# peteroh23/ModulationDetectionCNN

Measured on AMD Instinct MI355X. Metric: I/Q frames/sec (2x128, VT-CNN2, batch=2^20), higher is better.
Workload: dtype bf16; 1 GPU; vtcnn2-c11-bf16-n2^20; topology=vtcnn2, classes=11, frames_per_gpu=1048576, global_batch=1048576, parallelism=batch-shard x1 (no collective), outputs=softmax probabilities f32 + argmax int32, frames_per_forward_call=1048576, full=False

## Files before the change

### modulationdetectioncnn_amd/csrc/mdc_api.hip

```cpp
#include "mdc_internal.h"

#include <cstdlib>
#include <cstring>
#include <exception>
#include <mutex>
#include <new>

namespace mdc {

static thread_local char g_err[512] = "";

void set_error(const char* fmt, ...) {
    va_list ap;
    va_start(ap, fmt);
    vsnprintf(g_err, sizeof(g_err), fmt, ap);
    va_end(ap);
}

int upload(mdc_model* m, int idx, const void* host, size_t bytes) {
    if (m->d_pack[idx]) {
        (void)hipFree(m->d_pack[idx]);
        m->d_pack[idx] = nullptr;
    }
    MDC_HIP(hipMalloc(&m->d_pack[idx], bytes));
// ... 71 lines not shown
            return MDC_EINVAL;
    }
}

extern "C" {

int mdc_abi_version(void) { return MDC_ABI_VERSION; }

const char* mdc_last_error(void) { return g_err; }

int mdc_create(const mdc_topology* topo, int device, mdc_model** out) {
    return guarded("mdc_create", [&]() -> int {
        if (!topo || !out) { set_error("mdc_create: null argument"); return MDC_EINVAL; }
        *out = nullptr;
        if ((topo->reserved[0] & ~MDC_OPT_ALL) != 0) { set_error("mdc_create: unknown option bits 0x%x in reserved[0]", topo->reserved[0]); return MDC_EINVAL; }
        for (int i = 1; i < 4; ++i) if (topo->reserved[i] != 0) { set_error("mdc_create: reserved[1..3] must be 0"); return MDC_EINVAL; }
        if ((topo->reserved[0] & MDC_OPT_FP8_BF16_FEATURES) && topo->kind != MDC_KIND_VTCNN2) {
            set_error("mdc_create: MDC_OPT_FP8_BF16_FEATURES applies to MDC_KIND_VTCNN2 only");
            return MDC_EINVAL;
        }
        int ndev = 0;
        if (hipGetDeviceCount(&ndev) != hipSuccess || ndev == 0) { set_error("no HIP device available"); return MDC_ENODEV; }
        if (device < 0 || device >= ndev) { set_error("device %d out of range (have %d)", device, ndev); return MDC_ENODEV; }
        hipDeviceProp_t prop;
        MDC_HIP(hipGetDeviceProperties(&prop, device));
        if (std::strncmp(prop.gcnArchName, "gfx950", 6) != 0) {
            set_error("device %d is %s; libmdc.so carries gfx950 (MI355X) code only", device, prop.gcnArchName);
            return MDC_ENODEV;
        }
        mdc_model* m = new (std::nothrow) mdc_model();
        if (!m) { set_error("out of host memory"); return MDC_ENOMEM; }
        m->topo = *topo;
        m->device = device;
#ifdef MDC_ALTERNATES
        {
            auto flag = [](const char* name, int when) { const char* e = getenv(name); return e && atoi(e) == when; };
            if (flag("MDC_CONV_SCHED", 0)) m->alt |= kAltConvHipcc;
            if (flag("MDC_DENSE1_PHASED", 0)) m->alt |= kAltDense1Simple;
            if (flag("MDC_DEP_F32_MFMA", 1)) m->alt |= kAltDepF32Mfma;
            if (flag("MDC_D1_FUSED_HEAD", 0)) m->alt |= kAltSeparateHead;
            if (const char* e = getenv("MDC_DEP_RING")) m->alt_ring = atoi(e);
        }
#endif
        int rc = MDC_ENOMEM;
        try { rc = layer_layout(m); } catch (...) { delete m; throw; }
        if (rc != MDC_OK) { delete m; return rc; }
        *out = m;
        return MDC_OK;
    });
}

int mdc_num_layers(const mdc_model* m) {
    if (!m) { set_error("null model"); return MDC_EINVAL; }
    return m->nlayers;
}

int mdc_layer_sizes(const mdc_model* m, int layer, size_t* kernel_elems, size_t* bias_elems) {
    if (!m || layer < 0 || layer >= m->nlayers) { set_error("mdc_layer_sizes: bad layer %d", layer); return MDC_EINVAL; }
    if (kernel_elems) *kernel_elems = m->nk[layer];
    if (bias_elems) *bias_elems = m->nb[layer];
    return MDC_OK;
}

int mdc_set_weights(mdc_model* m, int layer, const float* kernel_host, size_t kernel_elems,
                    const float* bias_host, size_t bias_elems) {
    return guarded("mdc_set_weights", [&]() -> int {
        if (!m || !kernel_host || !bias_host) { set_error("mdc_set_weights: null argument"); return MDC_EINVAL; }
        if (m->finalized) { set_error("mdc_set_weights: model is finalized (immutable)"); return MDC_ESTATE; }
        if (layer < 0 || layer >= m->nlayers) { set_error("mdc_set_weights: layer %d out of range 0..%d", layer, m->nlayers - 1); return MDC_EINVAL; }
        if (kernel_elems != m->nk[layer] || bias_elems != m->nb[layer]) {
            set_error("mdc_set_weights: layer %d expects kernel %zu / bias %zu elements, got %zu / %zu",
                      layer, m->nk[layer], m->nb[layer], kernel_elems, bias_elems);
            return MDC_EINVAL;
        }
// ... 322 lines not shown
```

### modulationdetectioncnn_amd/csrc/mdc_internal.h

```cpp
#pragma once
#include <hip/hip_runtime.h>
#include <cstdarg>
#include <cstdint>
#include <cstdio>
#include <exception>
#include <mutex>
#include <new>
#include <string>
#include <type_traits>
#include <vector>

#include "mdc.h"

namespace mdc {

void set_error(const char* fmt, ...);

template <class Fn>
inline int guarded(const char* what, Fn&& fn) noexcept {
    try {
        return fn();
    } catch (const std::bad_alloc&) {
        set_error("%s: out of host memory", what);
        return MDC_ENOMEM;
// ... 55 lines not shown
    return max(max(__float_as_uint(v.x) & 0x7FFFFFFFu, __float_as_uint(v.y) & 0x7FFFFFFFu),
               max(__float_as_uint(v.z) & 0x7FFFFFFFu, __float_as_uint(v.w) & 0x7FFFFFFFu));
}

enum { kAltConvHipcc = 1,
       kAltDense1Simple = 2,
       kAltDepF32Mfma = 4,
       kAltSeparateHead = 8 };

struct ProfSlot {
    const char* name;
    std::vector<hipEvent_t> ev;
    double total_ms = 0;
    int64_t launches = 0;
};

}

struct mdc_model {
    mdc_topology topo{};
    int device = 0;
    int dtype = MDC_F32;
    bool finalized = false;
    int nlayers = 0;
    size_t nk[4]{}, nb[4]{};
    std::vector<float> hk[4], hb[4];
    bool have[4]{};

    void* d_pack[8]{};
    size_t pack_bytes[8]{};

    int alt = 0;
    int alt_ring = -1;
    float fp8_input_absmax = 0.02f;
    float fp8_feature_absmax = 0.f;
    int fp8_feat_scale_log2 = 0;
    bool fp8_e4m3_features = false;
    float fp8_feat_divisor = 1.f;
    int feat_scale_log2 = 0;

    bool profiling = false;
    std::vector<mdc::ProfSlot> slots;
    std::mutex prof_mu;

    void* host_ctx = nullptr;
    std::mutex host_mu;
};

namespace mdc {

struct ProfScope {
    mdc_model* m;
    int slot;
    hipStream_t s;
    hipEvent_t start = nullptr;
    ProfScope(const mdc_model* mm, int slot_, hipStream_t s_);
    ~ProfScope();
    ProfScope(const ProfScope&) = delete;
    ProfScope& operator=(const ProfScope&) = delete;
};

int upload(mdc_model* m, int idx, const void* host, size_t bytes);

struct DeviceScope {
    int prev = -1, want;
    bool ok = true;
// ... 67 lines not shown
```

### modulationdetectioncnn_amd/csrc/vtcnn2_bf16_common.h

```cpp
#pragma once
#include "mdc_internal.h"

#include <cstring>

namespace mdc {

using f32x4 = __attribute__((ext_vector_type(4))) float;
using f32x2 = __attribute__((ext_vector_type(2))) float;
using bf16x8 = __attribute__((ext_vector_type(8))) __bf16;
using bf16x2 = __attribute__((ext_vector_type(2))) __bf16;
using s16x4 = __attribute__((ext_vector_type(4))) short;
using s16x2 = __attribute__((ext_vector_type(2))) short;
using u32x4 = __attribute__((ext_vector_type(4))) unsigned;
using u32x2 = __attribute__((ext_vector_type(2))) unsigned;

namespace {

constexpr int kPairs = 67;
constexpr int kImgWords = 2 * kPairs * 64;
constexpr int kPartFloats = 4 * 5 * 64 * 4;
constexpr size_t kConvBf16Lds = (size_t)2 * kImgWords * 4 + (size_t)2 * kPartFloats * 4 + 512;
constexpr int kWFrags = 2 * 3 * 2 * 5;

__device__ __forceinline__ unsigned pack2(float a, float b) {
// ... 37 lines not shown
#pragma unroll
    for (int e = 0; e < 2; ++e) {
        const float a = xs[2 * e], b = xs[2 * e + 1];
        const unsigned hi = pack2(a, b);
        const float ah = __uint_as_float(hi << 16), bh = __uint_as_float(hi & 0xFFFF0000u);
        const unsigned lo = pack2(a - ah, b - bh);
        unsigned* d = im + (h * kPairs + 2 * m + 1 + e) * 64 + i;
        d[0] = hi;
        d[16] = lo;
        d[32] = hi;
    }
}
template <bool U8 = false>
__device__ __forceinline__ void stage_quarter(int k, const float* __restrict__ x, long n, long frame0,
                                              unsigned* __restrict__ im, int tid, long hop2 = 256, float scale = 0.f) {
    stage_write(k, stage_decode<U8>(stage_load<U8>(k, x, n, frame0, tid, hop2), tid, scale), n, frame0, im, tid);
}

__device__ __forceinline__ void glds16(const void* gsrc, void* lds_wave_base) {
    __builtin_amdgcn_global_load_lds((const __attribute__((address_space(1))) void*)gsrc,
                                     (__attribute__((address_space(3))) void*)lds_wave_base, 16, 0, 0);
}

__device__ __forceinline__ void glds16_nt(const void* gsrc, void* lds_wave_base) {
    __builtin_amdgcn_global_load_lds((const __attribute__((address_space(1))) void*)gsrc,
                                     (__attribute__((address_space(3))) void*)lds_wave_base, 16, 0, 2);
}

__device__ __forceinline__ void glds16_async(const void* gsrc, void* lds_wave_base) {
    const unsigned l = (unsigned)(size_t)(__attribute__((address_space(3))) unsigned char*)lds_wave_base;
    asm volatile("global_load_lds_dwordx4 %0, off" ::"v"(gsrc), "{m0}"(l) : "memory");
}

inline unsigned short f2bf(float f) {
    unsigned u;
    std::memcpy(&u, &f, 4);
    if ((u & 0x7F800000u) == 0x7F800000u) return (unsigned short)(u >> 16);
    u += 0x7FFFu + ((u >> 16) & 1u);
    return (unsigned short)(u >> 16);
}
inline float bf2f(unsigned short h) {
    unsigned u = (unsigned)h << 16;
    float f;
    std::memcpy(&f, &u, 4);
    return f;
}

}

int vtcnn2_bf16_conv_sched(const mdc_model* m, const float* x, int64_t n, void* feat, hipStream_t s, long hop2 = 0, float scale = 0.f);
int vtcnn2_bf16_pack_sched(mdc_model* m);

}
```

### modulationdetectioncnn_amd/csrc/vtcnn2_bf16_dense1.hip

```cpp
#include "vtcnn2_bf16_common.h"
#include "dense_chain_common.h"

#include <cstdlib>

namespace mdc {

namespace {

constexpr int kBM = 256, kBN = 256, kBK = 64;
constexpr int kTileBytes = kBM * kBK * 2;
constexpr size_t kDenseBf16Lds = (size_t)4 * kTileBytes;
constexpr size_t kDenseHeadLds = (size_t)128 * kChainXld * 4;
static_assert(kDenseHeadLds >= kDenseBf16Lds, "the fused-head form allocates the larger of the two");
constexpr int kNT = kFeat / kBK;

__device__ __forceinline__ bf16x8 cvt_e4m3x8(u32x2 r) {
    const bf16x2 p0 = __builtin_amdgcn_cvt_scalef32_pk_bf16_fp8(r[0], 1.0f, false);
    const bf16x2 p1 = __builtin_amdgcn_cvt_scalef32_pk_bf16_fp8(r[0], 1.0f, true);
    const bf16x2 p2 = __builtin_amdgcn_cvt_scalef32_pk_bf16_fp8(r[1], 1.0f, false);
    const bf16x2 p3 = __builtin_amdgcn_cvt_scalef32_pk_bf16_fp8(r[1], 1.0f, true);
    return bf16x8{p0[0], p0[1], p1[0], p1[1], p2[0], p2[1], p3[0], p3[1]};
}


#if defined(MDC_ALTERNATES) || defined(MDC_ABLATIONS)
template <int ABL>
__global__ __launch_bounds__(512) void vt_dense1_bf16_kernel(const unsigned short* __restrict__ feat, long n,
                                                             const unsigned short* __restrict__ w1t,
                                                             const float* __restrict__ c1,
                                                             float* __restrict__ hid) {
    extern __shared__ __attribute__((aligned(16))) unsigned char smem[];
    const int tid = threadIdx.x, lane = tid & 63;
    const int wv = __builtin_amdgcn_readfirstlane(tid >> 6);
    const int wr = wv >> 2, wc = wv & 3;
    const int fr = lane & 15, fg = lane >> 4;
    const long row0 = (long)blockIdx.x * kBM;

    const int srow = lane >> 3, spos = lane & 7;
    const unsigned short* asrc[4];
    const unsigned short* bsrc[4];
#pragma unroll
    for (int p = 0; p < 4; ++p) {
        const int r = (wv * 4 + p) * 8 + srow;
        long gr = (ABL == 1 ? 0 : row0) + r;
        if (gr >= n) gr = n - 1;
// ... 46 lines not shown
                for (int j = 0; j < 4; ++j)
                    acc[i][j] = __builtin_amdgcn_mfma_f32_16x16x32_bf16(af[i], bfr[j], acc[i][j], 0, 0, 0);
        }
    };

    stage(0, 0);
    __syncthreads();
    int cur = 0;
    for (int t = 0; t < kNT - 1; ++t) {
        stage(t + 1, cur ^ 1);
        compute(cur);
        __syncthreads();
        cur ^= 1;
    }
    compute(cur);

#pragma unroll
    for (int j = 0; j < 4; ++j) {
        const int col = wc * 64 + j * 16 + fr;
        const float bias = c1[col];
#pragma unroll
        for (int i = 0; i < 8; ++i)
#pragma unroll
            for (int r = 0; r < 4; ++r) {
                const long row = row0 + wr * 128 + i * 16 + fg * 4 + r;
                if (row < n) hid[row * kHid + col] = fmaxf(acc[i][j][r] + bias, 0.f);
            }
    }
}


#endif

template <bool HEAD>
__device__ __forceinline__ void d1_epilogue(f32x4 (&acc)[8][4], unsigned char* smem, long row0, long n, int lane, int wv,
                                            const float* __restrict__ c1, float* __restrict__ hid, const float* __restrict__ w2pack,
                                            int n_out, float* __restrict__ probs, int* __restrict__ labels) {
    const int wr = wv >> 2, wc = wv & 3, fr = lane & 15, fg = lane >> 4;
    if constexpr (!HEAD) {
#pragma unroll
        for (int j = 0; j < 4; ++j) {
            const int col = wc * 64 + j * 16 + fr;
            const float bias = c1[col];
#pragma unroll
            for (int i = 0; i < 8; ++i)
#pragma unroll
                for (int r = 0; r < 4; ++r) {
                    const long row = row0 + wr * 128 + i * 16 + fg * 4 + r;
                    if (row < n) hid[row * kHid + col] = fmaxf(acc[i][j][r] + bias, 0.f);
                }
        }
    } else {
        float* xs = reinterpret_cast<float*>(smem);
        float w2[64];
#pragma unroll
        for (int i = 0; i < 64; ++i) w2[i] = w2pack[i * 64 + lane];
        const float b2 = w2pack[64 * 64 + 16 * 64 + fr];
        float bias1[4];
#pragma unroll
        for (int j = 0; j < 4; ++j) bias1[j] = c1[wc * 64 + j * 16 + fr];
#pragma unroll
        for (int half = 0; half < 2; ++half) {
            __syncthreads();
            if (wr == half) {
#pragma unroll
                for (int j = 0; j < 4; ++j)
#pragma unroll
                    for (int i = 0; i < 8; ++i)
#pragma unroll
                        for (int r = 0; r < 4; ++r)
                            xs[(i * 16 + fg * 4 + r) * kChainXld + wc * 64 + j * 16 + fr] = fmaxf(acc[i][j][r] + bias1[j], 0.f);
            }
            __syncthreads();
            const f32x4 a2 = chain_k256(xs + (wv * 16 + fr) * kChainXld + fg, w2, f32x4{0.f, 0.f, 0.f, 0.f});
            f32x4 z;
#pragma unroll
            for (int r = 0; r < 4; ++r) z[r] = a2[r] + b2;
            chain_softmax_store(z, fr, fg, row0 + half * 128 + wv * 16, n, n_out, probs, labels, nullptr);
        }
    }
}

constexpr int kUnitBytes = 128 * 128;

template <int ABL, bool HEAD = false, bool F8 = false>
__global__ __launch_bounds__(512) void vt_dense1_bf16_phased_kernel(const unsigned short* __restrict__ feat, long n,
                                                                    const unsigned short* __restrict__ w1t,
                                                                    const float* __restrict__ c1, float* __restrict__ hid,
                                                                    const float* __restrict__ w2pack = nullptr, int n_out = 0,
                                                                    float* __restrict__ probs = nullptr, int* __restrict__ labels = nullptr) {
    extern __shared__ __attribute__((aligned(16))) unsigned char smem[];
    const int tid = threadIdx.x, lane = tid & 63;
    const int wv = __builtin_amdgcn_readfirstlane(tid >> 6);
    const int wr = wv >> 2, wc = wv & 3;
    const int fr = lane & 15, fg = lane >> 4;
    const long row0 = (long)blockIdx.x * kBM;

    const int srow = lane >> 3, spos = lane & 7;
    const unsigned short* src[4][2];
#pragma unroll
    for (int j = 0; j < 2; ++j) {
        const int u = (wv * 2 + j) * 8 + srow;
        const int sw = (spos ^ (u & 7)) * 8;
        const int arow_lo = 128 * (u >> 6) + (u & 63);
        const int brow_lo = 64 * (u >> 5) + (u & 31);
        long g0 = (ABL == 1 ? 0 : row0) + arow_lo, g3 = (ABL == 1 ? 0 : row0) + arow_lo + 64;
        if (g0 >= n) g0 = n - 1;
        if (g3 >= n) g3 = n - 1;
        src[0][j] = feat + g0 * (long)kFeat + sw;
        src[3][j] = feat + g3 * (long)kFeat + sw;
        src[1][j] = w1t + brow_lo * kBK + sw;
        src[2][j] = w1t + (brow_lo + 32) * kBK + sw;
    }
    const unsigned char* src8[2] = {nullptr, nullptr};
    if constexpr (F8) {
        const int u = wv * 16 + (lane >> 2);
        const int sw = ((lane & 3) ^ ((u >> 2) & 3)) * 16;
        const int arow_lo = 128 * (u >> 6) + (u & 63);
        long g0 = row0 + arow_lo, g3 = row0 + arow_lo + 64;
        if (g0 >= n) g0 = n - 1;
        if (g3 >= n) g3 = n - 1;
        const unsigned char* f8 = reinterpret_cast<const unsigned char*>(feat);
        src8[0] = f8 + g0 * (long)kFeat + sw;
        src8[1] = f8 + g3 * (long)kFeat + sw;
    }
    auto stage_unit = [&](int t, int unit, int b) {
        if (ABL == 2 && (unit == 1 || unit == 2) && (t & 1)) return;
        unsigned char* dst = smem + ((size_t)b * 4 + unit) * kUnitBytes + (wv * 2) * 1024;
        if constexpr (F8) {
            if (unit == 0 || unit == 3) {
                glds16(src8[unit == 3] + (long)t * kBK, smem + ((size_t)b * 4 + unit) * kUnitBytes + wv * 1024);
                return;
            }
        }
        if (unit == 0 || unit == 3) {
            glds16_nt(src[unit][0] + (long)t * kBK, dst);
            glds16_nt(src[unit][1] + (long)t * kBK, dst + 1024);
        } else {
            glds16(src[unit][0] + (long)t * (kBN * kBK), dst);
            glds16(src[unit][1] + (long)t * (kBN * kBK), dst + 1024);
        }
    };

    auto frag = [&](const unsigned char* unit_base, int u, int ks) {
        return *reinterpret_cast<const bf16x8*>(unit_base + u * 128 + (((ks * 4 + fg) ^ (u & 7)) * 16));
    };

    f32x4 acc[8][4];
#pragma unroll
    for (int i = 0; i < 8; ++i)
#pragma unroll
        for (int j = 0; j < 4; ++j) acc[i][j] = f32x4{0.f, 0.f, 0.f, 0.f};
    bf16x8 a0[4][2], a1[4][2], b0[2][2], b1[2][2];
    u32x2 ra[4][2];

    unsigned ra_lane[2] = {0u, 0u};
    if constexpr (F8) {
        ra_lane[0] = (unsigned)((64 * wr + fr) * 64 + ((((fg >> 1) ^ ((fr >> 2) & 3)) * 16) + (fg & 1) * 8));
        ra_lane[1] = ra_lane[0] ^ 32u;
    }
    auto read_a = [&](bf16x8 (&a)[4][2], int unit, int b) {
        if (ABL == 3 && b == 1) return;
        const unsigned char* base = smem + ((size_t)b * 4 + unit) * kUnitBytes;
        if constexpr (F8) {
            const unsigned bl = (unsigned)(size_t)(__attribute__((address_space(3))) unsigned char*)const_cast<unsigned char*>(base);
            const unsigned ad0 = bl + ra_lane[0], ad1 = bl + ra_lane[1];
#pragma unroll
            for (int i = 0; i < 4; ++i) {
                asm volatile("ds_read_b64 %0, %1 offset:%2" : "=v"(ra[i][0]) : "v"(ad0), "i"(i * 1024) : "memory");
                asm volatile("ds_read_b64 %0, %1 offset:%2" : "=v"(ra[i][1]) : "v"(ad1), "i"(i * 1024) : "memory");
            }
        } else {
#pragma unroll
            for (int i = 0; i < 4; ++i)
#pragma unroll
                for (int ks = 0; ks < 2; ++ks) a[i][ks] = frag(base, 64 * wr + 16 * i + fr, ks);
        }
    };
    auto cvt_a = [&](bf16x8 (&a)[4][2]) {
        if constexpr (F8) {
#pragma unroll
            for (int i = 0; i < 4; ++i)
#pragma unroll
                for (int ks = 0; ks < 2; ++ks) a[i][ks] = cvt_e4m3x8(ra[i][ks]);
        }
// ... 18 lines not shown
                for (int j = 0; j < 2; ++j)
                    acc[i0 + i][j0 + j] = __builtin_amdgcn_mfma_f32_16x16x32_bf16(a[i][ks], bq[j][ks], acc[i0 + i][j0 + j], 0, 0, 0);
#ifndef D1_NOPRIO
        __builtin_amdgcn_s_setprio(0);
#endif
    };
    auto quadrant_cv = [&](bf16x8 (&a)[4][2], const bf16x8 (&bq)[2][2], int i0, int j0, bf16x8 (&dst)[4][2], auto own) {
        constexpr bool OWN = decltype(own)::value;
        __builtin_amdgcn_s_setprio(1);
        if constexpr (OWN) a[0][0] = cvt_e4m3x8(ra[0][0]);
#pragma unroll
        for (int f = 0; f < 8; ++f) {
            const int ks = f >> 2, i = f & 3;
            if constexpr (OWN) { if (f + 1 < 8) a[(f + 1) & 3][(f + 1) >> 2] = cvt_e4m3x8(ra[(f + 1) & 3][(f + 1) >> 2]); }
            else dst[i][ks] = cvt_e4m3x8(ra[i][ks]);
#pragma unroll
            for (int j = 0; j < 2; ++j)
                acc[i0 + i][j0 + j] = __builtin_amdgcn_mfma_f32_16x16x32_bf16(a[i][ks], bq[j][ks], acc[i0 + i][j0 + j], 0, 0, 0);
        }
        if constexpr (OWN) __builtin_amdgcn_sched_group_barrier(0x002, 4, 0);
#pragma unroll
        for (int f = 0; f < 16; ++f) {
            __builtin_amdgcn_sched_group_barrier(0x008, 1, 0);
            __builtin_amdgcn_sched_group_barrier(0x002, 2, 0);
        }
        __builtin_amdgcn_s_setprio(0);
    };
#define D1_WAIT_BARRIER(N) do { asm volatile("s_waitcnt vmcnt(" #N ")" ::: "memory"); __builtin_amdgcn_s_barrier(); } while (0)
#define D1_LGKM() asm volatile("s_waitcnt lgkmcnt(0)" ::: "memory")
#define D1_LGKM_RA() asm volatile("s_waitcnt lgkmcnt(0)" : "+v"(ra[0][0]), "+v"(ra[0][1]), "+v"(ra[1][0]), "+v"(ra[1][1]), \
                                  "+v"(ra[2][0]), "+v"(ra[2][1]), "+v"(ra[3][0]), "+v"(ra[3][1]) :: "memory")

#pragma unroll
    for (int u = 0; u < 4; ++u) stage_unit(0, u, 0);
    D1_WAIT_BARRIER(0);
    read_a(a0, 0, 0);
    if constexpr (F8) { D1_LGKM_RA(); cvt_a(a0); }
#ifndef D1_NOSTAGGER
    if (wr == 1) __builtin_amdgcn_s_barrier();
#endif

    for (int t = 0; t < kNT; ++t) {
        const int b = t & 1;
        const bool more = t + 1 < kNT;
        if (more) stage_unit(t + 1, 0, b ^ 1);
        __builtin_amdgcn_sched_barrier(0);
        read_b(b0, 1, b);
        if constexpr (F8) { if (more) D1_WAIT_BARRIER(2); else D1_WAIT_BARRIER(1); }
        else { if (more) D1_WAIT_BARRIER(4); else D1_WAIT_BARRIER(2); }
        D1_LGKM();
        quadrant(a0, b0, 0, 0);
        __builtin_amdgcn_s_barrier();
        if (more) stage_unit(t + 1, 1, b ^ 1);
        __builtin_amdgcn_sched_barrier(0);
        read_b(b1, 2, b);
        if constexpr (F8) { if (more) D1_WAIT_BARRIER(3); else D1_WAIT_BARRIER(0); }
        else { if (more) D1_WAIT_BARRIER(4); else D1_WAIT_BARRIER(0); }
        D1_LGKM();
        quadrant(a0, b1, 0, 2);
        __builtin_amdgcn_s_barrier();
        if (more) stage_unit(t + 1, 2, b ^ 1);
        __builtin_amdgcn_sched_barrier(0);
        read_a(a1, 3, b);
        if (more) D1_WAIT_BARRIER(4); else __builtin_amdgcn_s_barrier();
        if constexpr (F8) { D1_LGKM_RA(); quadrant_cv(a1, b1, 4, 2, a1, std::true_type{}); }
        else { D1_LGKM(); quadrant(a1, b1, 4, 2); }
        __builtin_amdgcn_s_barrier();
        if (more) stage_unit(t + 1, 3, b ^ 1);
        __builtin_amdgcn_sched_barrier(0);
        if (more) read_a(a0, 0, b ^ 1);
        if constexpr (F8) { if (more) D1_WAIT_BARRIER(3); else __builtin_amdgcn_s_barrier(); }
        else { if (more) D1_WAIT_BARRIER(4); else __builtin_amdgcn_s_barrier(); }
        if constexpr (F8) {
            if (more) { D1_LGKM_RA(); quadrant_cv(a1, b0, 4, 0, a0, std::false_type{}); }
            else { D1_LGKM(); quadrant(a1, b0, 4, 0); }
        } else {
            quadrant(a1, b0, 4, 0);
            D1_LGKM();
        }
        __builtin_amdgcn_s_barrier();
    }
#ifndef D1_NOSTAGGER
    if (wr == 0) __builtin_amdgcn_s_barrier();
#endif
#undef D1_WAIT_BARRIER
#undef D1_LGKM
#undef D1_LGKM_RA

    d1_epilogue<HEAD>(acc, smem, row0, n, lane, wv, c1, hid, w2pack, n_out, probs, labels);
}


template <bool F8>
__global__ __launch_bounds__(64) void vt_dense1_bf16_small_kernel(const unsigned short* __restrict__ feat, long n,
                                                                  const unsigned short* __restrict__ w1t,
                                                                  const float* __restrict__ c1, float* __restrict__ hid) {
    const int lane = threadIdx.x, fr = lane & 15, fg = lane >> 4;
    const long row0 = (long)blockIdx.x * 16;
    const int col0 = blockIdx.y * 16;
    long ar = row0 + fr;
    if (ar >= n) ar = n - 1;
    using AFrag = typename std::conditional<F8, u32x2, bf16x8>::type;
    const unsigned char* ap = reinterpret_cast<const unsigned char*>(feat) + (ar * (long)kFeat + fg * 8) * (F8 ? 1 : 2);
    const unsigned short* bp = w1t + (long)(col0 + fr) * kBK + fg * 8;
    f32x4 acc = f32x4{0.f, 0.f, 0.f, 0.f};
    constexpr int kU = 5, kBlocks = kNT / kU;
    static_assert(kNT % kU == 0 && kBlocks % 2 == 1, "blocks: an even count in the loop, the last one drained after it");
    AFrag a0[kU][2], a1[kU][2];
    bf16x8 b0[kU][2], b1[kU][2];
    auto load = [&](AFrag (&af)[kU][2], bf16x8 (&bfr)[kU][2], int blk) {
#pragma unroll
        for (int u = 0; u < kU; ++u)
#pragma unroll
            for (int ks = 0; ks < 2; ++ks) {
                af[u][ks] = *reinterpret_cast<const AFrag*>(ap + ((blk * kU + u) * kBK + ks * 32) * (F8 ? 1 : 2));
                bfr[u][ks] = *reinterpret_cast<const bf16x8*>(bp + (long)(blk * kU + u) * (kBN * kBK) + ks * 32);
            }
    };
    auto mma = [&](const AFrag (&af)[kU][2], const bf16x8 (&bfr)[kU][2]) {
#pragma unroll
        for (int u = 0; u < kU; ++u)
#pragma unroll
            for (int ks = 0; ks < 2; ++ks) {
// ... 94 lines not shown
        asm volatile("s_waitcnt vmcnt(%0)\n\ts_barrier" ::"n"((kAhead - 1) * kGrp) : "memory");
        read(nxt, g + 1);
        mma(cur, kGrp);
        asm volatile("s_waitcnt lgkmcnt(0)" ::: "memory");
    };
    static_assert(kGroups % 2 == 1 && kTail >= 0 && kTail < kGrp, "pairs of steps, a last full group, then the tail tiles");
    for (int g = 0; g < kGroups - 1; g += 2) {
        step(f0, f1, g);
        step(f1, f0, g + 1);
    }
    step(f0, f1, kGroups - 1);
    mma(f1, kTail);
    asm volatile("s_waitcnt vmcnt(0)" ::: "memory");
    if (wv != 0) return;
    const int col = col0 + fr;
    const float bias = c1[col];
#pragma unroll
    for (int r = 0; r < 4; ++r) {
        const long row = row0 + fg * 4 + r;
        if (row < n) hid[row * kHid + col] = fmaxf(acc[r] + bias, 0.f);
    }
}

constexpr long kCoopBatch = 256;

constexpr long kSmallBatch = 2048;

}

int vtcnn2_bf16_dense1(const mdc_model* m, const void* feat, int64_t n, float* hid, hipStream_t s,
                       bool fuse_head, float* probs, int32_t* labels, bool* fused) {
    if (fused) *fused = false;
    const bool f8 = m->dtype == MDC_FP8 && m->fp8_e4m3_features;
    if (n <= kCoopBatch) {
#define MDC_LAUNCH_COOP(F) do { \
        MDC_HIP(hipFuncSetAttribute(reinterpret_cast<const void*>(vt_dense1_bf16_coop_kernel<F>), hipFuncAttributeMaxDynamicSharedMemorySize, (int)kCoopLds)); \
        hipLaunchKernelGGL(vt_dense1_bf16_coop_kernel<F>, dim3((unsigned)((n + 15) / 16), kHid / 16), dim3(256), kCoopLds, s, \
                           static_cast<const unsigned short*>(feat), (long)n, static_cast<const unsigned short*>(m->d_pack[3]), \
                           static_cast<const float*>(m->d_pack[4]), hid); } while (0)
        if (f8) MDC_LAUNCH_COOP(true); else MDC_LAUNCH_COOP(false);
#undef MDC_LAUNCH_COOP
        MDC_HIP(hipGetLastError());
        return MDC_OK;
    }
    if (n <= kSmallBatch) {
#define MDC_LAUNCH_SMALL(F) hipLaunchKernelGGL(vt_dense1_bf16_small_kernel<F>, dim3((unsigned)((n + 15) / 16), kHid / 16), dim3(64), 0, s, \
                           static_cast<const unsigned short*>(feat), (long)n, static_cast<const unsigned short*>(m->d_pack[3]), \
                           static_cast<const float*>(m->d_pack[4]), hid)
        if (f8) MDC_LAUNCH_SMALL(true); else MDC_LAUNCH_SMALL(false);
#undef MDC_LAUNCH_SMALL
        MDC_HIP(hipGetLastError());
        return MDC_OK;
    }
    const unsigned short* f = static_cast<const unsigned short*>(feat);
    const unsigned short* w1t = static_cast<const unsigned short*>(m->d_pack[3]);
    const float* c1 = static_cast<const float*>(m->d_pack[4]);
    const dim3 grid((unsigned)((n + kBM - 1) / kBM));
#if defined(MDC_ALTERNATES) || defined(MDC_ABLATIONS)
#define MDC_LAUNCH_D1(A) do { \
    MDC_HIP(hipFuncSetAttribute(reinterpret_cast<const void*>(vt_dense1_bf16_kernel<A>), hipFuncAttributeMaxDynamicSharedMemorySize, (int)kDenseBf16Lds)); \
    hipLaunchKernelGGL(vt_dense1_bf16_kernel<A>, grid, dim3(512), kDenseBf16Lds, s, f, (long)n, w1t, c1, hid); } while (0)
#endif
#ifdef MDC_ABLATIONS
    static const int abl = getenv("MDC_ABLATE_D1") ? atoi(getenv("MDC_ABLATE_D1")) : 0;
#define MDC_LAUNCH_PROBE(A) do { \
        MDC_HIP(hipFuncSetAttribute(reinterpret_cast<const void*>(vt_dense1_bf16_phased_kernel<A>), hipFuncAttributeMaxDynamicSharedMemorySize, (int)kDenseBf16Lds)); \
        hipLaunchKernelGGL(vt_dense1_bf16_phased_kernel<A>, grid, dim3(512), kDenseBf16Lds, s, f, (long)n, w1t, c1, hid); \
        MDC_HIP(hipGetLastError()); \
        return MDC_OK; } while (0)
    if (!f8 && abl == 10) MDC_LAUNCH_PROBE(0);
    if (!f8 && abl == 11) MDC_LAUNCH_PROBE(1);
    if (!f8 && abl == 12) MDC_LAUNCH_PROBE(2);
    if (!f8 && abl == 13) MDC_LAUNCH_PROBE(3);
#undef MDC_LAUNCH_PROBE
    if (abl >= 1 && abl <= 3) {
        switch (abl) { case 1: MDC_LAUNCH_D1(1); break; case 2: MDC_LAUNCH_D1(2); break; default: MDC_LAUNCH_D1(3); }
        MDC_HIP(hipGetLastError());
        return MDC_OK;
    }
#endif
#ifdef MDC_ALTERNATES
    if (!f8 && (m->alt & kAltDense1Simple)) {
        MDC_LAUNCH_D1(0);
        MDC_HIP(hipGetLastError());
        return MDC_OK;
    }
    if (m->alt & kAltSeparateHead) fuse_head = false;
#endif
#undef MDC_LAUNCH_D1
#define MDC_LAUNCH_PHASED(F) do { \
    if (fuse_head && (probs || labels)) { \
        MDC_HIP(hipFuncSetAttribute(reinterpret_cast<const void*>(vt_dense1_bf16_phased_kernel<0, true, F>), hipFuncAttributeMaxDynamicSharedMemorySize, (int)kDenseHeadLds)); \
        hipLaunchKernelGGL((vt_dense1_bf16_phased_kernel<0, true, F>), grid, dim3(512), kDenseHeadLds, s, f, (long)n, w1t, c1, hid, \
                           static_cast<const float*>(m->d_pack[5]), (int)m->topo.classes, probs, labels); \
        if (fused) *fused = true; \
    } else { \
        MDC_HIP(hipFuncSetAttribute(reinterpret_cast<const void*>(vt_dense1_bf16_phased_kernel<0, false, F>), hipFuncAttributeMaxDynamicSharedMemorySize, (int)kDenseBf16Lds)); \
        hipLaunchKernelGGL((vt_dense1_bf16_phased_kernel<0, false, F>), grid, dim3(512), kDenseBf16Lds, s, f, (long)n, w1t, c1, hid); \
    } } while (0)
    if (f8) MDC_LAUNCH_PHASED(true); else MDC_LAUNCH_PHASED(false);
#undef MDC_LAUNCH_PHASED
    MDC_HIP(hipGetLastError());
    return MDC_OK;
}

}
```

Measured before the change: 41.78 million frames/s.

## Make dense1 a persistent CU-sized grid that prefetches the next tile during the epilogue

The dense1 GEMM kernel now launches one workgroup per CU and loops over row tiles instead of launching one workgroup per tile. During each tile's epilogue it asynchronously issues the first k-tile loads for the next tile, using non-temporal loads for the feature rows, so the epilogue stores overlap the next tile's loads. The fused head stages W2, b2 and c1 into LDS once per workgroup and splits the head into four 64-row quarters handled by the first row of waves. This cuts per-tile launch and prologue cost, but a single workgroup per CU loses the latency hiding that multiple resident blocks gave, the reserved LDS grows, and only half the waves do head work.

```diff
diff --git a/modulationdetectioncnn_amd/csrc/mdc_api.hip b/modulationdetectioncnn_amd/csrc/mdc_api.hip
--- a/modulationdetectioncnn_amd/csrc/mdc_api.hip
+++ b/modulationdetectioncnn_amd/csrc/mdc_api.hip
@@ -127,6 +127,7 @@
         if (!m) { set_error("out of host memory"); return MDC_ENOMEM; }
         m->topo = *topo;
         m->device = device;
+        m->cu_count = prop.multiProcessorCount;
 #ifdef MDC_ALTERNATES
         {
             auto flag = [](const char* name, int when) { const char* e = getenv(name); return e && atoi(e) == when; };
@@ -135,6 +136,7 @@
             if (flag("MDC_DEP_F32_MFMA", 1)) m->alt |= kAltDepF32Mfma;
             if (flag("MDC_D1_FUSED_HEAD", 0)) m->alt |= kAltSeparateHead;
             if (const char* e = getenv("MDC_DEP_RING")) m->alt_ring = atoi(e);
+            if (const char* e = getenv("MDC_D1_GRID")) m->alt_d1_grid = atoi(e) > 0 ? atoi(e) : 0;
         }
 #endif
         int rc = MDC_ENOMEM;
diff --git a/modulationdetectioncnn_amd/csrc/mdc_internal.h b/modulationdetectioncnn_amd/csrc/mdc_internal.h
--- a/modulationdetectioncnn_amd/csrc/mdc_internal.h
+++ b/modulationdetectioncnn_amd/csrc/mdc_internal.h
@@ -111,6 +111,8 @@
 
     int alt = 0;
     int alt_ring = -1;
+    int alt_d1_grid = 0;
+    int cu_count = 0;
     float fp8_input_absmax = 0.02f;
     float fp8_feature_absmax = 0.f;
     int fp8_feat_scale_log2 = 0;
diff --git a/modulationdetectioncnn_amd/csrc/vtcnn2_bf16_common.h b/modulationdetectioncnn_amd/csrc/vtcnn2_bf16_common.h
--- a/modulationdetectioncnn_amd/csrc/vtcnn2_bf16_common.h
+++ b/modulationdetectioncnn_amd/csrc/vtcnn2_bf16_common.h
@@ -93,6 +93,11 @@
     asm volatile("global_load_lds_dwordx4 %0, off" ::"v"(gsrc), "{m0}"(l) : "memory");
 }
 
+__device__ __forceinline__ void glds16_async_nt(const void* gsrc, void* lds_wave_base) {
+    const unsigned l = (unsigned)(size_t)(__attribute__((address_space(3))) unsigned char*)lds_wave_base;
+    asm volatile("global_load_lds_dwordx4 %0, off nt" ::"v"(gsrc), "{m0}"(l) : "memory");
+}
+
 inline unsigned short f2bf(float f) {
     unsigned u;
     std::memcpy(&u, &f, 4);
diff --git a/modulationdetectioncnn_amd/csrc/vtcnn2_bf16_dense1.hip b/modulationdetectioncnn_amd/csrc/vtcnn2_bf16_dense1.hip
--- a/modulationdetectioncnn_amd/csrc/vtcnn2_bf16_dense1.hip
+++ b/modulationdetectioncnn_amd/csrc/vtcnn2_bf16_dense1.hip
@@ -10,7 +10,10 @@
 constexpr int kBM = 256, kBN = 256, kBK = 64;
 constexpr int kTileBytes = kBM * kBK * 2;
 constexpr size_t kDenseBf16Lds = (size_t)4 * kTileBytes;
-constexpr size_t kDenseHeadLds = (size_t)128 * kChainXld * 4;
+constexpr size_t kDenseHeadOff = (size_t)2 * kTileBytes;
+constexpr size_t kDenseHeadConstOff = kDenseHeadOff + (size_t)64 * kChainXld * 4;
+constexpr int kHeadW2 = 64 * 64, kHeadB2 = 16;
+constexpr size_t kDenseHeadLds = kDenseHeadConstOff + (size_t)(kHeadW2 + kHeadB2 + kHid) * 4;
 static_assert(kDenseHeadLds >= kDenseBf16Lds, "the fused-head form allocates the larger of the two");
 constexpr int kNT = kFeat / kBK;
 
@@ -123,99 +126,126 @@
 
 #endif
 
-template <bool HEAD>
+__device__ __forceinline__ void d1_head_consts(unsigned char* smem, int tid, const float* __restrict__ c1, const float* __restrict__ w2pack) {
+    float* cs = reinterpret_cast<float*>(smem + kDenseHeadConstOff);
+#pragma unroll
+    for (int i = 0; i < kHeadW2 / 512; ++i) cs[i * 512 + tid] = w2pack[i * 512 + tid];
+    if (tid < kHeadB2) cs[kHeadW2 + tid] = w2pack[64 * 64 + 16 * 64 + tid];
+    if (tid < kHid) cs[kHeadW2 + kHeadB2 + tid] = c1[tid];
+    asm volatile("s_waitcnt lgkmcnt(0)" ::: "memory");
+}
+
+template <bool HEAD, class Prefetch>
 __device__ __forceinline__ void d1_epilogue(f32x4 (&acc)[8][4], unsigned char* smem, long row0, long n, int lane, int wv,
                                             const float* __restrict__ c1, float* __restrict__ hid, const float* __restrict__ w2pack,
-                                            int n_out, float* __restrict__ probs, int* __restrict__ labels) {
+                                            int n_out, float* __restrict__ probs, int* __restrict__ labels, Prefetch&& prefetch) {
     const int wr = wv >> 2, wc = wv & 3, fr = lane & 15, fg = lane >> 4;
+    float bias1[4];
     if constexpr (!HEAD) {
+#pragma unroll
+        for (int j = 0; j < 4; ++j) bias1[j] = c1[wc * 64 + j * 16 + fr];
+        asm volatile("" : "+v"(bias1[0]), "+v"(bias1[1]), "+v"(bias1[2]), "+v"(bias1[3]));
+        prefetch();
 #pragma unroll
         for (int j = 0; j < 4; ++j) {
             const int col = wc * 64 + j * 16 + fr;
-            const float bias = c1[col];
 #pragma unroll
             for (int i = 0; i < 8; ++i)
 #pragma unroll
                 for (int r = 0; r < 4; ++r) {
                     const long row = row0 + wr * 128 + i * 16 + fg * 4 + r;
-                    if (row < n) hid[row * kHid + col] = fmaxf(acc[i][j][r] + bias, 0.f);
+                    if (row < n) hid[row * kHid + col] = fmaxf(acc[i][j][r] + bias1[j], 0.f);
                 }
         }
     } else {
-        float* xs = reinterpret_cast<float*>(smem);
+        prefetch();
+        float* xs = reinterpret_cast<float*>(smem + kDenseHeadOff);
+        const float* cs = reinterpret_cast<const float*>(smem + kDenseHeadConstOff);
+#pragma unroll
+        for (int j = 0; j < 4; ++j) bias1[j] = cs[kHeadW2 + kHeadB2 + wc * 64 + j * 16 + fr];
         float w2[64];
-#pragma unroll
-        for (int i = 0; i < 64; ++i) w2[i] = w2pack[i * 64 + lane];
-        const float b2 = w2pack[64 * 64 + 16 * 64 + fr];
-        float bias1[4];
-#pragma unroll
-        for (int j = 0; j < 4; ++j) bias1[j] = c1[wc * 64 + j * 16 + fr];
-#pragma unroll
-        for (int half = 0; half < 2; ++half) {
-            __syncthreads();
-            if (wr == half) {
+        float b2 = 0.f;
+        if (wr == 0) {
+#pragma unroll
+            for (int i = 0; i < 64; ++i) w2[i] = cs[i * 64 + lane];
+            b2 = cs[kHeadW2 + fr];
+        }
+#pragma unroll
+        for (int q = 0; q < 4; ++q) {
+            if (q > 0) asm volatile("s_barrier" ::: "memory");
+            if (wr == (q >> 1)) {
 #pragma unroll
                 for (int j = 0; j < 4; ++j)
 #pragma unroll
-                    for (int i = 0; i < 8; ++i)
+                    for (int i = 0; i < 4; ++i)
 #pragma unroll
                         for (int r = 0; r < 4; ++r)
-                            xs[(i * 16 + fg * 4 + r) * kChainXld + wc * 64 + j * 16 + fr] = fmaxf(acc[i][j][r] + bias1[j], 0.f);
-            }
-            __syncthreads();
-            const f32x4 a2 = chain_k256(xs + (wv * 16 + fr) * kChainXld + fg, w2, f32x4{0.f, 0.f, 0.f, 0.f});
-            f32x4 z;
-#pragma unroll
-            for (int r = 0; r < 4; ++r) z[r] = a2[r] + b2;
-            chain_softmax_store(z, fr, fg, row0 + half * 128 + wv * 16, n, n_out, probs, labels, nullptr);
+                            xs[(i * 16 + fg * 4 + r) * kChainXld + wc * 64 + j * 16 + fr] = fmaxf(acc[4 * (q & 1) + i][j][r] + bias1[j], 0.f);
+            }
+            asm volatile("s_waitcnt lgkmcnt(0)\n\ts_barrier" ::: "memory");
+            if (wr == 0) {
+                const f32x4 a2 = chain_k256(xs + (wv * 16 + fr) * kChainXld + fg, w2, f32x4{0.f, 0.f, 0.f, 0.f});
+                f32x4 z;
+#pragma unroll
+                for (int r = 0; r < 4; ++r) z[r] = a2[r] + b2;
+                chain_softmax_store(z, fr, fg, row0 + q * 64 + wv * 16, n, n_out, probs, labels, nullptr);
+            }
         }
     }
 }
 
 constexpr int kUnitBytes = 128 * 128;
 
-template <int ABL, bool HEAD = false, bool F8 = false>
-__global__ __launch_bounds__(512) void vt_dense1_bf16_phased_kernel(const unsigned short* __restrict__ feat, long n,
-                                                                    const unsigned short* __restrict__ w1t,
-                                                                    const float* __restrict__ c1, float* __restrict__ hid,
-                                                                    const float* __restrict__ w2pack = nullptr, int n_out = 0,
-                                                                    float* __restrict__ probs = nullptr, int* __restrict__ labels = nullptr) {
-    extern __shared__ __attribute__((aligned(16))) unsigned char smem[];
-    const int tid = threadIdx.x, lane = tid & 63;
-    const int wv = __builtin_amdgcn_readfirstlane(tid >> 6);
-    const int wr = wv >> 2, wc = wv & 3;
-    const int fr = lane & 15, fg = lane >> 4;
-    const long row0 = (long)blockIdx.x * kBM;
-
-    const int srow = lane >> 3, spos = lane & 7;
+__device__ __forceinline__ int d1_lane() {
+    int l;
+    asm volatile("v_mbcnt_lo_u32_b32 %0, -1, 0\n\tv_mbcnt_hi_u32_b32 %0, -1, %0" : "=v"(l));
+    return l;
+}
+
+template <int ABL, bool F8>
+struct D1Stage {
     const unsigned short* src[4][2];
-#pragma unroll
-    for (int j = 0; j < 2; ++j) {
-        const int u = (wv * 2 + j) * 8 + srow;
-        const int sw = (spos ^ (u & 7)) * 8;
-        const int arow_lo = 128 * (u >> 6) + (u & 63);
-        const int brow_lo = 64 * (u >> 5) + (u & 31);
-        long g0 = (ABL == 1 ? 0 : row0) + arow_lo, g3 = (ABL == 1 ? 0 : row0) + arow_lo + 64;
-        if (g0 >= n) g0 = n - 1;
-        if (g3 >= n) g3 = n - 1;
-        src[0][j] = feat + g0 * (long)kFeat + sw;
-        src[3][j] = feat + g3 * (long)kFeat + sw;
-        src[1][j] = w1t + brow_lo * kBK + sw;
-        src[2][j] = w1t + (brow_lo + 32) * kBK + sw;
-    }
-    const unsigned char* src8[2] = {nullptr, nullptr};
-    if constexpr (F8) {
-        const int u = wv * 16 + (lane >> 2);
-        const int sw = ((lane & 3) ^ ((u >> 2) & 3)) * 16;
-        const int arow_lo = 128 * (u >> 6) + (u & 63);
-        long g0 = row0 + arow_lo, g3 = row0 + arow_lo + 64;
-        if (g0 >= n) g0 = n - 1;
-        if (g3 >= n) g3 = n - 1;
-        const unsigned char* f8 = reinterpret_cast<const unsigned char*>(feat);
-        src8[0] = f8 + g0 * (long)kFeat + sw;
-        src8[1] = f8 + g3 * (long)kFeat + sw;
-    }
-    auto stage_unit = [&](int t, int unit, int b) {
+    const unsigned char* src8[2];
+    __device__ __forceinline__ D1Stage(const unsigned short* __restrict__ feat, const unsigned short* __restrict__ w1t, long n, long row0, int lane, int wv) {
+        const int srow = lane >> 3, spos = lane & 7;
+#pragma unroll
+        for (int j = 0; j < 2; ++j) {
+            const int u = (wv * 2 + j) * 8 + srow;
+            const int sw = (spos ^ (u & 7)) * 8;
+            const int arow_lo = 128 * (u >> 6) + (u & 63);
+            const int brow_lo = 64 * (u >> 5) + (u & 31);
+            long g0 = (ABL == 1 ? 0 : row0) + arow_lo, g3 = (ABL == 1 ? 0 : row0) + arow_lo + 64;
+            if (g0 >= n) g0 = n - 1;
+            if (g3 >= n) g3 = n - 1;
+            src[0][j] = feat + g0 * (long)kFeat + sw;
+            src[3][j] = feat + g3 * (long)kFeat + sw;
+            src[1][j] = w1t + brow_lo * kBK + sw;
+            src[2][j] = w1t + (brow_lo + 32) * kBK + sw;
+        }
+        src8[0] = src8[1] = nullptr;
+        if constexpr (F8) {
+            const int u = wv * 16 + (lane >> 2);
+            const int sw = ((lane & 3) ^ ((u >> 2) & 3)) * 16;
+            const int arow_lo = 128 * (u >> 6) + (u & 63);
+            long g0 = row0 + arow_lo, g3 = row0 + arow_lo + 64;
+            if (g0 >= n) g0 = n - 1;
+            if (g3 >= n) g3 = n - 1;
+            const unsigned char* f8 = reinterpret_cast<const unsigned char*>(feat);
+            src8[0] = f8 + g0 * (long)kFeat + sw;
+            src8[1] = f8 + g3 * (long)kFeat + sw;
+        }
+    }
+    __device__ __forceinline__ void ktile0_async(unsigned char* smem, int wv) const {
+#pragma unroll
+        for (int u = 0; u < 4; ++u) {
+            unsigned char* dst = smem + (size_t)u * kUnitBytes + (wv * 2) * 1024;
+            const bool a = u == 0 || u == 3;
+            if (F8 && a) { glds16_async(src8[u == 3], smem + (size_t)u * kUnitBytes + wv * 1024); continue; }
+            if (a) { glds16_async_nt(src[u][0], dst); glds16_async_nt(src[u][1], dst + 1024); }
+            else { glds16_async(src[u][0], dst); glds16_async(src[u][1], dst + 1024); }
+        }
+    }
+    __device__ __forceinline__ void unit(int t, int unit, int b, unsigned char* smem, int wv) const {
         if (ABL == 2 && (unit == 1 || unit == 2) && (t & 1)) return;
         unsigned char* dst = smem + ((size_t)b * 4 + unit) * kUnitBytes + (wv * 2) * 1024;
         if constexpr (F8) {
@@ -231,17 +261,61 @@
             glds16(src[unit][0] + (long)t * (kBN * kBK), dst);
             glds16(src[unit][1] + (long)t * (kBN * kBK), dst + 1024);
         }
-    };
+    }
+    __device__ __forceinline__ void ktile0(unsigned char* smem, int wv) const {
+#pragma unroll
+        for (int u = 0; u < 4; ++u) unit(0, u, 0, smem, wv);
+    }
+};
+
+#ifdef MDC_ABLATIONS
+#define D1_STAMP_PARAM , unsigned long long* __restrict__ stamps = nullptr
+#define D1_STAMP(K) do { if (stamps) d1_ts[K] = __builtin_amdgcn_s_memrealtime(); } while (0)
+#define D1_STAMP_TILE() do { if (stamps) { \
+        D1_STAMP(3); \
+        if (wv == 0 && d1_lane() == 0) { \
+            unsigned long long* o = stamps + tile * 8; \
+            o[0] = d1_ts[0]; o[1] = d1_ts[1]; o[2] = d1_ts[2]; o[3] = d1_ts[3]; \
+            o[4] = ((unsigned long long)__builtin_amdgcn_s_getreg((3 << 11) | 20) << 32) | __builtin_amdgcn_s_getreg((31 << 11) | 4);   \
+            o[5] = blockIdx.x; \
+        } \
+        d1_ts[0] = d1_ts[3]; } } while (0)
+#else
+#define D1_STAMP_PARAM
+#define D1_STAMP(K) do { } while (0)
+#define D1_STAMP_TILE() do { } while (0)
+#endif
+template <int ABL, bool HEAD = false, bool F8 = false>
+__global__ __launch_bounds__(512) void vt_dense1_bf16_phased_kernel(const unsigned short* __restrict__ feat, long n,
+                                                                    const unsigned short* __restrict__ w1t,
+                                                                    const float* __restrict__ c1, float* __restrict__ hid,
+                                                                    const float* __restrict__ w2pack = nullptr, int n_out = 0,
+                                                                    float* __restrict__ probs = nullptr, int* __restrict__ labels = nullptr
+                                                                    D1_STAMP_PARAM) {
+    extern __shared__ __attribute__((aligned(16))) unsigned char smem[];
+    const int tid = threadIdx.x;
+    const int wv = __builtin_amdgcn_readfirstlane(tid >> 6);
+    const int wr = wv >> 2, wc = wv & 3;
+    const long ntiles = (n + kBM - 1) / kBM;
+#ifdef MDC_ABLATIONS
+    unsigned long long d1_ts[4] = {0, 0, 0, 0};
+#endif
+    D1_STAMP(0);
+
+    D1Stage<ABL, F8>(feat, w1t, n, (long)blockIdx.x * kBM, d1_lane(), wv).ktile0(smem, wv);
+    if constexpr (HEAD) d1_head_consts(smem, tid, c1, w2pack);
+    for (long tile = blockIdx.x; tile < ntiles; tile += gridDim.x) {
+    const long row0 = tile * kBM;
+    const int lane = d1_lane();
+    const int fr = lane & 15, fg = lane >> 4;
+    const D1Stage<ABL, F8> st(feat, w1t, n, row0, lane, wv);
+    auto stage_unit = [&](int t, int unit, int b) { st.unit(t, unit, b, smem, wv); };
 
     auto frag = [&](const unsigned char* unit_base, int u, int ks) {
         return *reinterpret_cast<const bf16x8*>(unit_base + u * 128 + (((ks * 4 + fg) ^ (u & 7)) * 16));
     };
 
     f32x4 acc[8][4];
-#pragma unroll
-    for (int i = 0; i < 8; ++i)
-#pragma unroll
-        for (int j = 0; j < 4; ++j) acc[i][j] = f32x4{0.f, 0.f, 0.f, 0.f};
     bf16x8 a0[4][2], a1[4][2], b0[2][2], b1[2][2];
     u32x2 ra[4][2];
 
@@ -326,8 +400,11 @@
                                   "+v"(ra[2][0]), "+v"(ra[2][1]), "+v"(ra[3][0]), "+v"(ra[3][1]) :: "memory")
 
 #pragma unroll
-    for (int u = 0; u < 4; ++u) stage_unit(0, u, 0);
+    for (int i = 0; i < 8; ++i)
+#pragma unroll
+        for (int j = 0; j < 4; ++j) acc[i][j] = f32x4{0.f, 0.f, 0.f, 0.f};
     D1_WAIT_BARRIER(0);
+    D1_STAMP(1);
     read_a(a0, 0, 0);
     if constexpr (F8) { D1_LGKM_RA(); cvt_a(a0); }
 #ifndef D1_NOSTAGGER
@@ -377,12 +454,20 @@
 #ifndef D1_NOSTAGGER
     if (wr == 0) __builtin_amdgcn_s_barrier();
 #endif
+    D1_STAMP(2);
+    const long next = tile + gridDim.x;
+    d1_epilogue<HEAD>(acc, smem, row0, n, d1_lane(), wv, c1, hid, w2pack, n_out, probs, labels, [&]() {
+        if (next < ntiles) D1Stage<ABL, F8>(feat, w1t, n, next * kBM, d1_lane(), wv).ktile0_async(smem, wv);
+    });
+    D1_STAMP_TILE();
+    }
 #undef D1_WAIT_BARRIER
 #undef D1_LGKM
 #undef D1_LGKM_RA
-
-    d1_epilogue<HEAD>(acc, smem, row0, n, lane, wv, c1, hid, w2pack, n_out, probs, labels);
-}
+}
+#undef D1_STAMP_PARAM
+#undef D1_STAMP
+#undef D1_STAMP_TILE
 
 
 template <bool F8>
@@ -543,7 +628,11 @@
                        bool fuse_head, float* probs, int32_t* labels, bool* fused) {
     if (fused) *fused = false;
     const bool f8 = m->dtype == MDC_FP8 && m->fp8_e4m3_features;
-    if (n <= kCoopBatch) {
+    bool tiled = n > kSmallBatch;
+#ifdef MDC_ALTERNATES
+    if (m->alt_d1_grid > 0) tiled = true;
+#endif
+    if (!tiled && n <= kCoopBatch) {
 #define MDC_LAUNCH_COOP(F) do { \
         MDC_HIP(hipFuncSetAttribute(reinterpret_cast<const void*>(vt_dense1_bf16_coop_kernel<F>), hipFuncAttributeMaxDynamicSharedMemorySize, (int)kCoopLds)); \
         hipLaunchKernelGGL(vt_dense1_bf16_coop_kernel<F>, dim3((unsigned)((n + 15) / 16), kHid / 16), dim3(256), kCoopLds, s, \
@@ -554,7 +643,7 @@
         MDC_HIP(hipGetLastError());
         return MDC_OK;
     }
-    if (n <= kSmallBatch) {
+    if (!tiled) {
 #define MDC_LAUNCH_SMALL(F) hipLaunchKernelGGL(vt_dense1_bf16_small_kernel<F>, dim3((unsigned)((n + 15) / 16), kHid / 16), dim3(64), 0, s, \
                            static_cast<const unsigned short*>(feat), (long)n, static_cast<const unsigned short*>(m->d_pack[3]), \
                            static_cast<const float*>(m->d_pack[4]), hid)
@@ -566,11 +655,17 @@
     const unsigned short* f = static_cast<const unsigned short*>(feat);
     const unsigned short* w1t = static_cast<const unsigned short*>(m->d_pack[3]);
     const float* c1 = static_cast<const float*>(m->d_pack[4]);
-    const dim3 grid((unsigned)((n + kBM - 1) / kBM));
+    const long tiles = (long)((n + kBM - 1) / kBM);
+    if (m->cu_count <= 0) { set_error("vtcnn2_bf16_dense1: the model does not know its device's CU count"); return MDC_ESTATE; }
+    long walkers = tiles < m->cu_count ? tiles : (long)m->cu_count;
+#ifdef MDC_ALTERNATES
+    if (m->alt_d1_grid > 0 && walkers > m->alt_d1_grid) walkers = m->alt_d1_grid;
+#endif
+    const dim3 grid((unsigned)walkers);
 #if defined(MDC_ALTERNATES) || defined(MDC_ABLATIONS)
 #define MDC_LAUNCH_D1(A) do { \
     MDC_HIP(hipFuncSetAttribute(reinterpret_cast<const void*>(vt_dense1_bf16_kernel<A>), hipFuncAttributeMaxDynamicSharedMemorySize, (int)kDenseBf16Lds)); \
-    hipLaunchKernelGGL(vt_dense1_bf16_kernel<A>, grid, dim3(512), kDenseBf16Lds, s, f, (long)n, w1t, c1, hid); } while (0)
+    hipLaunchKernelGGL(vt_dense1_bf16_kernel<A>, dim3((unsigned)tiles), dim3(512), kDenseBf16Lds, s, f, (long)n, w1t, c1, hid); } while (0)
 #endif
 #ifdef MDC_ABLATIONS
     static const int abl = getenv("MDC_ABLATE_D1") ? atoi(getenv("MDC_ABLATE_D1")) : 0;
@@ -599,19 +694,46 @@
     if (m->alt & kAltSeparateHead) fuse_head = false;
 #endif
 #undef MDC_LAUNCH_D1
+#ifdef MDC_ABLATIONS
+    const char* stamp_path = getenv("MDC_D1_STAMPS");
+    const bool one_tile = getenv("MDC_D1_ONE_TILE") && atoi(getenv("MDC_D1_ONE_TILE")) == 1;
+    const dim3 grid_s(one_tile ? (unsigned)tiles : grid.x);
+    unsigned long long* stamps = nullptr;
+    if (stamp_path) {
+        MDC_HIP(hipMalloc(reinterpret_cast<void**>(&stamps), (size_t)tiles * 64));
+        MDC_HIP(hipMemsetAsync(stamps, 0, (size_t)tiles * 64, s));
+    }
+#define D1_GRID grid_s
+#define D1_STAMP_ARG , stamps
+#else
+#define D1_GRID grid
+#define D1_STAMP_ARG
+#endif
 #define MDC_LAUNCH_PHASED(F) do { \
     if (fuse_head && (probs || labels)) { \
         MDC_HIP(hipFuncSetAttribute(reinterpret_cast<const void*>(vt_dense1_bf16_phased_kernel<0, true, F>), hipFuncAttributeMaxDynamicSharedMemorySize, (int)kDenseHeadLds)); \
-        hipLaunchKernelGGL((vt_dense1_bf16_phased_kernel<0, true, F>), grid, dim3(512), kDenseHeadLds, s, f, (long)n, w1t, c1, hid, \
-                           static_cast<const float*>(m->d_pack[5]), (int)m->topo.classes, probs, labels); \
+        hipLaunchKernelGGL((vt_dense1_bf16_phased_kernel<0, true, F>), D1_GRID, dim3(512), kDenseHeadLds, s, f, (long)n, w1t, c1, hid, \
+                           static_cast<const float*>(m->d_pack[5]), (int)m->topo.classes, probs, labels D1_STAMP_ARG); \
         if (fused) *fused = true; \
     } else { \
         MDC_HIP(hipFuncSetAttribute(reinterpret_cast<const void*>(vt_dense1_bf16_phased_kernel<0, false, F>), hipFuncAttributeMaxDynamicSharedMemorySize, (int)kDenseBf16Lds)); \
-        hipLaunchKernelGGL((vt_dense1_bf16_phased_kernel<0, false, F>), grid, dim3(512), kDenseBf16Lds, s, f, (long)n, w1t, c1, hid); \
+        hipLaunchKernelGGL((vt_dense1_bf16_phased_kernel<0, false, F>), D1_GRID, dim3(512), kDenseBf16Lds, s, f, (long)n, w1t, c1, hid, \
+                           static_cast<const float*>(nullptr), 0, static_cast<float*>(nullptr), static_cast<int*>(nullptr) D1_STAMP_ARG); \
     } } while (0)
     if (f8) MDC_LAUNCH_PHASED(true); else MDC_LAUNCH_PHASED(false);
 #undef MDC_LAUNCH_PHASED
+#undef D1_GRID
+#undef D1_STAMP_ARG
     MDC_HIP(hipGetLastError());
+#ifdef MDC_ABLATIONS
+    if (stamps) {
+        std::vector<unsigned long long> host((size_t)tiles * 8);
+        MDC_HIP(hipStreamSynchronize(s));
+        MDC_HIP(hipMemcpy(host.data(), stamps, host.size() * 8, hipMemcpyDeviceToHost));
+        MDC_HIP(hipFree(stamps));
+        if (FILE* fp = fopen(stamp_path, "wb")) { fwrite(host.data(), 8, host.size(), fp); fclose(fp); }
+    }
+#endif
     return MDC_OK;
 }
 
```

After: 41.65 million frames/s. About the same (-0.3%).
